# shanglianlm0525/CvPytorch

Measured on AMD Instinct MI355X. Metric: images/sec/node train step, YOLOv5-s@640 (value: batch resident in HBM when the timed region starts; with_h2d.value: the same step fed from pinned host memory inside the region) & DeepLabv3+R50@1024x512 (config3_deeplabv3plus_r50.value), higher is better.
Workload: dtype bf16; 1 GPU; coco_yolov5_s.yml YOLOv5-s 640x640 bf16 train step (fwd+loss+bwd+SGD-nesterov+EMA), per-GPU batch 64, synthetic COCO-shape tensors resident in HBM; global_batch=64, parallelism=dp1, launch=hipGraph replay of the whole step, world=1, transport=none (single process), grad_buckets=0, sync_bn=False, deterministic=True

## Files before the change

### cvpytorch_amd/csrc/conv1x1_stream.hip

```cpp
#include <stdlib.h>

#include "common.h"
#include "conv_plan.h"

namespace cvhip {

constexpr int kS1MaxLds = 72 * 1024;
constexpr int kS1MaxBlocks = 512;
constexpr int kS1MinTiles = 192;


template <int NV>
__device__ __forceinline__ void s1_act_vec(float (&v)[NV], int act, float ap) {
  switch (act) {
    case CVHIP_ACT_NONE: break;
    case CVHIP_ACT_RELU:
#pragma unroll
      for (int q = 0; q < NV; ++q) v[q] = act_fwd(v[q], CVHIP_ACT_RELU, ap);
      break;
    case CVHIP_ACT_SILU:
#pragma unroll
      for (int q = 0; q < NV; ++q) v[q] = act_fwd(v[q], CVHIP_ACT_SILU, ap);
      break;
    case CVHIP_ACT_LEAKY:
#pragma unroll
      for (int q = 0; q < NV; ++q) v[q] = act_fwd(v[q], CVHIP_ACT_LEAKY, ap);
      break;
    case CVHIP_ACT_SIGMOID:
#pragma unroll
      for (int q = 0; q < NV; ++q) v[q] = act_fwd(v[q], CVHIP_ACT_SIGMOID, ap);
      break;
    default:
#pragma unroll
      for (int q = 0; q < NV; ++q) v[q] = act_fwd(v[q], CVHIP_ACT_HSWISH, ap);
      break;
  }
}

template <int NF, int MF, int STATS, bool EPI = false, bool PRO = false>
__global__ __launch_bounds__(256, 2) void conv1x1_stream_kernel(const IgemmKernArgs p, int ntiles, int vec16) {
  constexpr int BN = NF * 16;
  constexpr int RT = 64 * MF;
  constexpr int KC = 256 / MF;
  constexpr int KS = KC / 32;
  extern __shared__ __attribute__((aligned(16))) unsigned char smem[];

  const int t = threadIdx.x;
  const int lane = t & 63;
  const int wave = __builtin_amdgcn_readfirstlane(t >> 6);
  const int r = lane & 15, g = lane >> 4;
  const int Cin = p.Cin;
  const int M = p.cls[0].M;
  const int cin_pad = (Cin + 31) & ~31;
  const int brow = cin_pad * 2 + 16;
  const int nkc = (cin_pad + KC - 1) / KC;
  const int n0 = blockIdx.y * BN;

  const int my_tiles = (ntiles - (int)blockIdx.x + (int)gridDim.x - 1) / (int)gridDim.x;
  const int total = my_tiles * nkc;

  h16x8 buf0[MF][KS], buf1[MF][KS];

  int ld_tile = blockIdx.x, ld_kc = 0;
  auto load = [&](h16x8 (&dst)[MF][KS]) {
    const int row0 = ld_tile * RT + wave * (MF * 16) + r;
    const int kbase = ld_kc * KC + g * 8;
#pragma unroll
    for (int b = 0; b < MF; ++b) {
      int m = row0 + b * 16;
      m = m < M ? m : M - 1;
      const h16_t* src = p.x + (int64_t)m * p.x_ld;
#pragma unroll
      for (int ks = 0; ks < KS; ++ks) {
        int kk = kbase + ks * 32;
        kk = kk < Cin ? kk : 0;
        dst[b][ks] = *reinterpret_cast<const h16x8*>(src + kk);
      }
    }
    if (++ld_kc == nkc) {
      ld_kc = 0;
      ld_tile += gridDim.x;
    }
  };

  load(buf0);

  {
    const int cpr = cin_pad >> 3;
    const int nchunks = BN * cpr;
    constexpr int U = 8;
    for (int q0 = t; q0 < nchunks; q0 += 256 * U) {
      uint4 v[U];
      int dst[U];
#pragma unroll
      for (int u = 0; u < U; ++u) {
        const int q = q0 + u * 256;
        const int L = q / cpr;
        const int kq = q - L * cpr;
        const int a = L >> 4, i = L & 15;
        const int ch = n0 + (a >> 1) * 32 + (i >> 2) * 8 + (a & 1) * 4 + (i & 3);
        dst[u] = q < nchunks ? L * brow + kq * 16 : -1;
        v[u] = make_uint4(0u, 0u, 0u, 0u);
        if (q < nchunks && ch < p.Nout && kq * 8 < Cin) v[u] = *reinterpret_cast<const uint4*>(p.w + (int64_t)ch * Cin + kq * 8);
      }
#pragma unroll
      for (int u = 0; u < U; ++u)
        if (dst[u] >= 0) *reinterpret_cast<uint4*>(smem + dst[u]) = v[u];
    }
  }
  float* const sbias = reinterpret_cast<float*>(smem + BN * brow);
  const float* const sepi = sbias + BN;
  if (p.bias && t < BN) sbias[t] = (n0 + t < p.bias_n) ? p.bias[n0 + t] : 0.f;
  static_assert(!EPI || STATS == 0, "the fused epilogue excludes BatchNorm sums");
  if (EPI && t < BN) {
    const int n = n0 + t < p.Nout ? n0 + t : p.Nout - 1;
    sbias[BN + t] = p.ep_scale ? p.ep_scale[n] : 1.f;
    sbias[2 * BN + t] = p.ep_scale ? p.ep_shift[n] : 0.f;
  }
  float* const spro = sbias + 5 * BN;
  if constexpr (PRO) {
    for (int c = t; c < cin_pad; c += 256) {
      const bool in = c >= p.pro_lo && c < p.pro_hi && c < Cin;
      spro[c] = in ? p.pro_scale[c] : 1.f;
      spro[cin_pad + c] = in ? p.pro_shift[c] : 0.f;
    }
  }
  __syncthreads();

  f32x4 acc[NF][MF];
#pragma unroll
  for (int a = 0; a < NF; ++a)
#pragma unroll
    for (int b = 0; b < MF; ++b) acc[a][b] = f32x4{0.f, 0.f, 0.f, 0.f};
  float s1[STATS ? NF : 1][4], s2[STATS ? NF : 1][4];
  if constexpr (STATS) {
#pragma unroll
    for (int a = 0; a < NF; ++a)
#pragma unroll
      for (int q = 0; q < 4; ++q) s1[a][q] = s2[a][q] = 0.f;
  }

  const unsigned char* const wlane = smem + r * brow + g * 16;
  int cp_tile = blockIdx.x, cp_kc = 0;
  auto compute = [&](const h16x8 (&src)[MF][KS]) {
    const unsigned char* wk = wlane + cp_kc * (KC * 2);
    const int ksn = min(KS, (cin_pad - cp_kc * KC) >> 5);
#pragma unroll
    for (int ks = 0; ks < KS; ++ks) {
      if (ks < ksn) {
#pragma unroll
        for (int a = 0; a < NF; ++a) {
          const h16x8 wb = *reinterpret_cast<const h16x8*>(wk + a * 16 * brow + ks * 64);
#pragma unroll
          for (int b = 0; b < MF; ++b) acc[a][b] = CVHIP_MFMA_16X16X32(wb, src[b][ks], acc[a][b], 0, 0, 0);
        }
      }
    }
    if (++cp_kc < nkc) return;
    const int row0 = cp_tile * RT + wave * (MF * 16) + r;
#pragma unroll
    for (int b = 0; b < MF; ++b) {
      const int m = row0 + b * 16;
      h16_t* yrow = p.y + (int64_t)m * p.y_ld;
#pragma unroll
      for (int j = 0; j < NF / 2; ++j) {
        const int ch0 = n0 + j * 32 + g * 8;
        f32x8 v;
#pragma unroll
        for (int q = 0; q < 4; ++q) {
          v.v[q] = acc[2 * j][b][q];
          v.v[4 + q] = acc[2 * j + 1][b][q];
        }
        if constexpr (STATS == 1) {
          const float keep = m < M ? 1.f : 0.f;
#pragma unroll
          for (int q = 0; q < 8; ++q) v.v[q] *= keep;
#pragma unroll
          for (int q = 0; q < 4; ++q) {
            s1[2 * j][q] += v.v[q];
            s2[2 * j][q] += v.v[q] * v.v[q];
            s1[2 * j + 1][q] += v.v[4 + q];
            s2[2 * j + 1][q] += v.v[4 + q] * v.v[4 + q];
          }
        }
        if (p.bias) {
          const f32x4 b0 = *reinterpret_cast<const f32x4*>(sbias + j * 32 + g * 8);
          const f32x4 b1 = *reinterpret_cast<const f32x4*>(sbias + j * 32 + g * 8 + 4);
#pragma unroll
          for (int q = 0; q < 4; ++q) {
            v.v[q] += b0[q];
            v.v[4 + q] += b1[q];
          }
        }
        if constexpr (EPI) {
          const int cl8 = j * 32 + g * 8;
#pragma unroll
          for (int q = 0; q < 8; ++q) v.v[q] = v.v[q] * sepi[cl8 + q] + sepi[BN + cl8 + q];
          if (p.res && p.res_pre && m < M) {
            const h16_t* rrow = p.res + (int64_t)m * p.res_ld + ch0;
#pragma unroll
            for (int q = 0; q < 8; ++q)
              if (ch0 + q < p.Nout) v.v[q] += (float)rrow[q];
          }
          s1_act_vec<8>(v.v, p.ep_act, p.ep_ap);
        }
        if (p.res && !(EPI && p.res_pre) && m < M) {
          const h16_t* rrow = p.res + (int64_t)m * p.res_ld + ch0;
          if (ch0 + 7 < p.Nout && (p.res_ld & 7) == 0 && ((((uintptr_t)p.res) & 15) == 0)) {
            const f32x8 rv = unpack8(*reinterpret_cast<const uint4*>(rrow));
#pragma unroll
            for (int q = 0; q < 8; ++q) v.v[q] += rv.v[q];
          } else {
#pragma unroll
            for (int q = 0; q < 8; ++q)
              if (ch0 + q < p.Nout) v.v[q] += (float)rrow[q];
          }
        }
        if (m < M) {
          h16_t* const dst = (p.y2 && ch0 >= p.y_split) ? p.y2 + (int64_t)m * p.y2_ld + (ch0 - p.y_split) : yrow + ch0;
          if (vec16 && ch0 + 7 < p.Nout) {
            *reinterpret_cast<uint4*>(dst) = pack8(v);
          } else {
#pragma unroll
            for (int q = 0; q < 8; ++q)
              if (ch0 + q < p.Nout) dst[q] = (h16_t)v.v[q];
          }
        }
      }
    }
#pragma unroll
    for (int a = 0; a < NF; ++a)
#pragma unroll
      for (int b = 0; b < MF; ++b) acc[a][b] = f32x4{0.f, 0.f, 0.f, 0.f};
    cp_kc = 0;
    cp_tile += gridDim.x;
  };

  auto xform = [&](h16x8 (&buf)[MF][KS]) {
    const int kbase = cp_kc * KC + g * 8;
    const int ksn = min(KS, (cin_pad - cp_kc * KC) >> 5);
#pragma unroll
    for (int ks = 0; ks < KS; ++ks) {
      int kk = kbase + ks * 32;
      kk = kk < Cin ? kk : 0;
      if (ks < ksn && kk >= p.pro_lo && kk < p.pro_hi) {
        const f32x4 c0 = *reinterpret_cast<const f32x4*>(spro + kk), c1 = *reinterpret_cast<const f32x4*>(spro + kk + 4);
        const f32x4 h0 = *reinterpret_cast<const f32x4*>(spro + cin_pad + kk), h1 = *reinterpret_cast<const f32x4*>(spro + cin_pad + kk + 4);
#pragma unroll
        for (int b = 0; b < MF; ++b) {
          f32x8 v = unpack8(__builtin_bit_cast(uint4, buf[b][ks]));
#pragma unroll
          for (int q = 0; q < 4; ++q) {
            v.v[q] = v.v[q] * c0[q] + h0[q];
            v.v[4 + q] = v.v[4 + q] * c1[q] + h1[q];
          }
          s1_act_vec<8>(v.v, p.pro_act, p.pro_ap);
          buf[b][ks] = __builtin_bit_cast(h16x8, pack8(v));
        }
      }
    }
  };

  for (int it = 0; it < total; it += 2) {
    load(buf1);
    if constexpr (PRO) xform(buf0);
    compute(buf0);
    load(buf0);
    if constexpr (PRO) xform(buf1);
    compute(buf1);
  }

  if constexpr (STATS) {
    if (p.stats) {
      __syncthreads();
      float* red = reinterpret_cast<float*>(smem);
#pragma unroll
      for (int a = 0; a < NF; ++a)
#pragma unroll
        for (int q = 0; q < 4; ++q) {
          const float u1 = row16_sum(s1[a][q]), u2 = row16_sum(s2[a][q]);
          if (r == 0) {
            const int lc = (a >> 1) * 32 + g * 8 + (a & 1) * 4 + q;
            red[(wave * BN + lc) * 2 + 0] = u1;
            red[(wave * BN + lc) * 2 + 1] = u2;
          }
        }
      __syncthreads();
      if (t < BN && n0 + t < p.Nout) {
        float u1 = 0.f, u2 = 0.f;
#pragma unroll
        for (int w = 0; w < 4; ++w) {
          u1 += red[(w * BN + t) * 2 + 0];
          u2 += red[(w * BN + t) * 2 + 1];
        }
        if (p.stats_acc) {
          acc_add2(reinterpret_cast<double*>(p.stats), blockIdx.x, p.stats_ld, n0 + t, u1, u2);
        } else {
          float* dst = p.stats + (int64_t)blockIdx.x * 2 * p.Nout;
          dst[n0 + t] = u1;
          dst[p.Nout + n0 + t] = u2;
        }
      }
    }
  }
}


static int s1x1_mode() {
  static int v = -1;
  if (v < 0) {
    const char* e = getenv("CVHIP_S1X1");
    v = e ? atoi(e) : 1;
  }
  return v;
}

static int s1x1_nf(int Nout, int Cin, bool stats) {
  if (Nout <= 32) return 2;
  if (Nout <= 64) return 4;
  if (Nout > 128 && Nout <= 256 && !stats && 256 * (((Cin + 31) & ~31) * 2 + 16) <= kS1MaxLds) return 16;
  return 8;
}

int stream1x1_blocks(int Nout, int Cin, int64_t M, bool stats) {
  const int mode = s1x1_mode();
  if (mode == 0 || (Cin & 7) || M <= 0 || M >= (1ll << 31)) return 0;
  const int bn = s1x1_nf(Nout, Cin, stats) * 16;
  const int cin_pad = (Cin + 31) & ~31;
  if (bn * (cin_pad * 2 + 16) > kS1MaxLds) return 0;
  const int ntiles = (int)((M + 127) / 128);
  if (mode == 1) {
    if (ntiles < kS1MinTiles) return 0;
    if (Nout > bn && (Nout > 4 * bn || stats || (double)M * Cin * 2.0 > 64e6)) return 0;
  }
  const int max_blocks = kS1MaxBlocks;
  const int rounds = cdiv(ntiles, max_blocks);
  return cdiv(ntiles, rounds);
}

static bool s1x1_structural(const IgemmParams& p) {
  if (p.ncls != 1) return false;
  const IgemmClass& c = p.cls[0];
  return c.TR == 1 && c.TS == 1 && p.in_sh == 1 && p.in_sw == 1 && p.out_sh == 1 && p.out_sw == 1 && c.dh0 == 0 && c.dw0 == 0 &&
         c.out_oh == 0 && c.out_ow == 0 && c.OHi == p.OH && c.OWi == p.OW && p.IH == p.OH && p.IW == p.OW && (p.x_ld & 7) == 0;
}

static int s1x1_lds(int bn, int cin_pad, bool pro) {
  int lds = bn * (cin_pad * 2 + 16) + 5 * bn * (int)sizeof(float) + (pro ? 2 * cin_pad * (int)sizeof(float) : 0);
  if (lds < 4 * bn * 2 * (int)sizeof(float)) lds = 4 * bn * 2 * (int)sizeof(float);
  return lds;
}
constexpr int kS1MaxLdsPro = kS1MaxLds + 4096;

template <int NF, int STATS, bool EPI = false, bool PRO = false>
static int launch_s1(const IgemmParams& p, int blocks, int ntiles, hipStream_t stream) {
  constexpr int MF = 2;
  const int bn = NF * 16;
  const int cin_pad = (p.Cin + 31) & ~31;
  const int lds = s1x1_lds(bn, cin_pad, PRO);
  if (lds > kS1MaxLdsPro) return CVHIP_ERR_UNSUPPORTED;
  auto kern = conv1x1_stream_kernel<NF, MF, STATS, EPI, PRO>;
  static bool attr_done[64] = {};
  int devid = 0;
  (void)hipGetDevice(&devid);
  bool& attr_set = attr_done[devid & 63];
  if (!attr_set) {
    hipError_t e = hipFuncSetAttribute(reinterpret_cast<const void*>(kern), hipFuncAttributeMaxDynamicSharedMemorySize, kS1MaxLds + 4096);
    if (e != hipSuccess) {
      set_last_error("hipFuncSetAttribute(conv1x1_stream_kernel)", e);
      return CVHIP_ERR_LAUNCH;
    }
    attr_set = true;
  }
  const int vec16 = ((p.y_ld & 7) == 0) && ((((uintptr_t)p.y) & 15) == 0);
  const IgemmKernArgs k = narrow_plan(p, 0, 1);
  hipLaunchKernelGGL(kern, dim3(blocks, cdiv(p.Nout, bn)), dim3(256), lds, stream, k, ntiles, vec16);
  return check_launch("conv1x1_stream_kernel");
}

bool stream1x1_prologue_ok(const IgemmParams& p, bool stats) {
  if (!s1x1_structural(p)) return false;
  if (stream1x1_blocks(p.Nout, p.Cin, p.cls[0].M, stats) <= 0) return false;
  const int nf = s1x1_nf(p.Nout, p.Cin, stats);
  if (nf == 16) return false;
  return s1x1_lds(nf * 16, (p.Cin + 31) & ~31, true) <= kS1MaxLdsPro;
}

int try_launch_stream1x1(const IgemmParams& p, hipStream_t stream) {
  if (!s1x1_structural(p)) return -1;
  const int64_t M = p.cls[0].M;
  const int blocks = stream1x1_blocks(p.Nout, p.Cin, M, p.stats != nullptr);
  if (blocks <= 0) return -1;
  const int ntiles = (int)((M + 127) / 128);
  const int nf = s1x1_nf(p.Nout, p.Cin, p.stats != nullptr);
  if (p.stats && (p.ep_scale || p.ep_act != CVHIP_ACT_NONE)) return CVHIP_ERR_INVALID;
  if (p.z_out) return CVHIP_ERR_UNSUPPORTED;
  if (p.y2 && ((p.y_split & 7) || p.y_split <= 0 || p.y_split >= p.Nout || (p.y2_ld & 7) || (((uintptr_t)p.y2) & 15) || (p.y_ld & 7) ||
               (((uintptr_t)p.y) & 15) || (p.Nout & 7)))
    return CVHIP_ERR_INVALID;
  if (p.pro_scale) {
    if (p.ep_scale || p.ep_act != CVHIP_ACT_NONE || p.res || !stream1x1_prologue_ok(p, p.stats != nullptr)) return CVHIP_ERR_UNSUPPORTED;
    if (p.pro_lo < 0 || p.pro_hi > p.Cin || p.pro_lo >= p.pro_hi || (p.pro_lo & 7) || (p.pro_hi & 7)) return CVHIP_ERR_INVALID;
    if (p.stats) {
      if (nf == 2) return launch_s1<2, 1, false, true>(p, blocks, ntiles, stream);
      if (nf == 4) return launch_s1<4, 1, false, true>(p, blocks, ntiles, stream);
      return launch_s1<8, 1, false, true>(p, blocks, ntiles, stream);
    }
    if (nf == 2) return launch_s1<2, 0, false, true>(p, blocks, ntiles, stream);
    if (nf == 4) return launch_s1<4, 0, false, true>(p, blocks, ntiles, stream);
    return launch_s1<8, 0, false, true>(p, blocks, ntiles, stream);
  }
  if (p.stats) {
    if (nf == 2) return launch_s1<2, 1>(p, blocks, ntiles, stream);
    if (nf == 4) return launch_s1<4, 1>(p, blocks, ntiles, stream);
    return launch_s1<8, 1>(p, blocks, ntiles, stream);
  }
  if (p.ep_scale || p.ep_act != CVHIP_ACT_NONE) {
    if (nf == 2) return launch_s1<2, 0, true>(p, blocks, ntiles, stream);
    if (nf == 4) return launch_s1<4, 0, true>(p, blocks, ntiles, stream);
    if (nf == 16) return launch_s1<16, 0, true>(p, blocks, ntiles, stream);
    return launch_s1<8, 0, true>(p, blocks, ntiles, stream);
  }
  if (nf == 2) return launch_s1<2, 0>(p, blocks, ntiles, stream);
  if (nf == 4) return launch_s1<4, 0>(p, blocks, ntiles, stream);
  if (nf == 16) return launch_s1<16, 0>(p, blocks, ntiles, stream);
  return launch_s1<8, 0>(p, blocks, ntiles, stream);
}

}
```

### cvpytorch_amd/ops.py

```python
import ctypes as C

import torch

from . import lib as L

ACT_DTYPE = torch.bfloat16
_weights_epoch = 0
_stats_epoch = [0]


def set_precision(p):
    global ACT_DTYPE
    L.set_precision(p)
    ACT_DTYPE = torch.float16 if p == "fp16" else torch.bfloat16
    bump_weights_epoch()
    _desc_cache.clear()


def precision():
    return L.PRECISION


def bump_weights_epoch():
    global _weights_epoch
    _weights_epoch += 1


_STEM_IMAGE = __import__("os").environ.get("CVHIP_STEM_IMAGE", "1") != "0"
_EPI_FUSE = __import__("os").environ.get("CVHIP_EPI_FUSE", "1") != "0"
_BN_ACC = __import__("os").environ.get("CVHIP_BN_ACC", "1") != "0"
_DW_STATS = __import__("os").environ.get("CVHIP_DW_STATS", "1") != "0"
_BN_ACC_MAX_C = 2048
_acc_epoch = 0


_DETERMINISTIC = __import__("os").environ.get("CVHIP_DETERMINISTIC", "0") == "1"


def set_deterministic(flag=True):
    global _DETERMINISTIC
    _DETERMINISTIC = bool(flag)


def is_deterministic():
    return _DETERMINISTIC


def _wgrad(kname, geom, desc, x, dy, dst, accumulate, st):
    if _DETERMINISTIC:
        nb = L.load().cvhip_conv2d_wgrad_det_workspace_bytes(C.byref(desc))
        if nb < 0:
            L.check(int(nb), "cvhip_conv2d_wgrad_det_workspace_bytes")
        ws = torch.empty((max(int(nb), 16),), dtype=torch.uint8, device=x.device)
        _timed_call(kname, geom, "cvhip_conv2d_wgrad_det", C.byref(desc), x.data_ptr(), dy.data_ptr(), dst.data_ptr(), int(accumulate),
                    ws.data_ptr(), int(nb), st)
    else:
        _timed_call(kname, geom, "cvhip_conv2d_wgrad", C.byref(desc), x.data_ptr(), dy.data_ptr(), dst.data_ptr(), int(accumulate), st)


def bump_acc_epoch():
    global _acc_epoch
    _acc_epoch += 1


def _layer_acc(cfg, K, dev):
    owner = cfg.acc_owner
    if owner is not None:
        ent = owner.__dict__.get(cfg.acc_attr)
        if ent is not None and len(ent) >= 4 and ent[3] == id(owner) and ent[1] != ent[2][0] and ent[0].shape[-1] == K and ent[0].device == dev:
            ent[1] = ent[2][0]
            return ent[0][0], ent[0][1]
    t = zero_fill(torch.empty((2, L.BN_ACC_SHARDS, 2, K), dtype=torch.float64, device=dev))
    return t[0], t[1]


def _stream():
    return torch.cuda.current_stream().cuda_stream


_LAZY = __import__("os").environ.get("CVHIP_LAZY", "1") != "0"
_LAZY_ACTS = (L.ACT_NONE, L.ACT_RELU, L.ACT_LEAKY, L.ACT_SILU)


_OWNED_BACKWARD = [False]


def set_lazy(flag=True):
    global _LAZY
    _LAZY = bool(flag)


class LazyAct:
    __slots__ = ("scale", "shift", "act", "ap", "z", "lo", "hi")

    def __init__(self, scale, shift, act, ap, lo=0, hi=None):
        self.scale, self.shift, self.act, self.ap = scale, shift, int(act), float(ap)
        self.lo = int(lo)
        self.hi = int(hi) if hi is not None else self.lo + int(scale.numel())
        self.z = None

    def full(self, Cc):
        return self.lo == 0 and self.hi == Cc

    def scale_ptr(self):
        return self.scale.data_ptr() - 4 * self.lo

    def shift_ptr(self):
        return self.shift.data_ptr() - 4 * self.lo


def act_id_of(conv_module):
    fus = conv_module._fusable(True, True) if hasattr(conv_module, "_fusable") else None
    return fus[1][0] if fus is not None else -1


def lazy_of(t):
    return getattr(t, "_hip_lazy", None) if t is not None else None


_LAZY_META = frozenset((
    "size", "stride", "dim", "ndimension", "numel", "nelement", "data_ptr", "storage_offset", "is_contiguous", "element_size", "__len__",
    "shape", "device", "dtype", "is_cuda", "requires_grad", "grad_fn", "is_leaf", "layout", "names", "ndim", "_version", "_base", "grad",
    "is_floating_point", "is_complex", "get_device", "is_sparse", "is_quantized", "is_meta", "untyped_storage", "_is_view", "output_nr",
    "register_hook", "retain_grad", "retains_grad", "__hash__", "__repr__", "__format__", "_backward_hooks", "is_pinned", "is_shared"))


class LazyRaw(torch.Tensor):

    @classmethod
    def __torch_function__(cls, func, types, args=(), kwargs=None):
        kwargs = kwargs or {}
        name = getattr(func, "__name__", "")
        if name == "__get__" or name == "__set__":
            name = getattr(getattr(func, "__self__", None), "__name__", name)
        if name in _LAZY_META:
            with torch._C.DisableTorchFunctionSubclass():
                return func(*args, **kwargs)
        from torch.utils._pytree import tree_map

        def fix(a):
            if isinstance(a, LazyRaw):
                with torch._C.DisableTorchFunctionSubclass():
                    return materialize(a) if lazy_of(a) is not None else a.as_subclass(torch.Tensor)
            return a

        args, kwargs = tree_map(fix, args), tree_map(fix, kwargs)
        with torch._C.DisableTorchFunctionSubclass():
            return func(*args, **kwargs)


def tag_lazy(t, lz):
    with torch._C.DisableTorchFunctionSubclass():
        z = t.as_subclass(LazyRaw)
    z._hip_lazy = lz
    return z


class Materialize(torch.autograd.Function):

    @staticmethod
    def forward(ctx, y, lz):
        yy, y_ld = as_nhwc(y, lazy_ok=True)
        N, K, P, Q = yy.shape
        z = empty_nhwc(N, K, P, Q, yy.device)
        _materialize_into(yy, y_ld, z, K, lz)
        return z

    @staticmethod
    def backward(ctx, dz):
        return dz, None


def _materialize_into(x, x_ld, z, z_ld, lz):
    N, Cc, H, W = x.shape
    M = N * H * W
    st = _stream()
    if not lz.full(Cc):
        L.call("cvhip_copy2d", x.data_ptr(), x_ld, z.data_ptr(), z_ld, M, Cc, st)
    kh = lz.hi - lz.lo
    _timed_ew("bn_act_fwd(ew_kernel<0>)", 4.0 * M * kh, "cvhip_bn_act_fwd", x.data_ptr() + 2 * lz.lo, x_ld, z.data_ptr() + 2 * lz.lo, z_ld, M, kh,
              lz.scale.data_ptr(), lz.shift.data_ptr(), lz.act, lz.ap, None, 0, st)


def materialize(x):
    lz = lazy_of(x)
    if lz is None:
        return x
    if lz.z is None:
        lz.z = Materialize.apply(x, lz)
    return lz.z


def _lazy_in(lz):
    return L.LazyIn(lz.scale_ptr(), lz.shift_ptr(), lz.act, lz.ap, lz.lo, lz.hi)


class KernelTimer:

    def __init__(self):
        self.enabled = False
        self.records = []
        self.detail = []

    def reset(self):
        self.records = []
        self.detail = []

    def summary(self):
        out = {}
        for name, fl, by, e0, e1 in self.records:
            d = out.setdefault(name, dict(launches=0, ms=0.0, flops=0.0, bytes=0.0))
            d["launches"] += 1
            d["ms"] += e0.elapsed_time(e1)
            d["flops"] += fl
            d["bytes"] += by
        return out


TIMER = KernelTimer()


def _igemm_name(nout, m=0, ktot=0, pointwise=False, ld=0, stats=False):
    if pointwise and ld % 8 == 0 and L.load().cvhip_conv1x1_stream_blocks(nout, ktot, m, int(stats)) > 0:
        wide = nout > 128 and not stats and 256 * (((ktot + 31) // 32 * 32) * 2 + 16) <= 72 * 1024 and nout <= 256
        return "conv1x1_stream_kernel<%d>" % (32 if nout <= 32 else 64 if nout <= 64 else 256 if wide else 128)
    if nout <= 32:
        return "igemm_kernel<256,32,64,32>"
    if nout <= 64:
        return "igemm_kernel<256,64,64,64>"
    big = ktot >= 512 and ((m + 255) // 256) * ((nout + 127) // 128) >= 384
    return "igemm_kernel<256,128,128,64>" if big else "igemm_kernel<128,128,64,64>"


def _pointwise(R, S, cfg):
    return R == 1 and S == 1 and tuple(cfg.stride) == (1, 1) and tuple(cfg.pad) == (0, 0)


def _wgrad_name(k, r=3, s=3, c=0, m=0, desc=None):
    if desc is not None and L.load().cvhip_conv_stem_blocks(C.byref(desc)) > 0 and desc.y_ld % 8 == 0:
        return "stem_wgrad_kernel"
    tn = 32 if k <= 32 else 64 if k <= 64 else 128
    if r == 1 and s == 1 and float(m) * k * c <= 7.5e9:
        if k >= 256 and c >= 256:
            return "wgrad_kernel<128,64,64,2>"
        tn = 32
    return {32: "wgrad_kernel<32,32,32>", 64: "wgrad_kernel<64,32,64>", 128: "wgrad_kernel<128,64,64>"}[tn]


def _timed_call(kname, geom, fname, *args, passes=1, nbytes=None):
    if not TIMER.enabled:
        L.call(fname, *args)
        return
    N, Cc, H, W, K, R, S, P, Q = geom
    flops = 2.0 * N * P * Q * K * R * S * Cc * passes
    if nbytes is None:
        nbytes = 2.0 * (N * H * W * Cc + N * P * Q * K + K * R * S * Cc)
    if kname.startswith("igemm_kernel") and (fname.startswith("cvhip_conv2d_fprop") or fname.startswith("cvhip_conv2d_dgrad")):
        try:
            dg = 1 if fname.startswith("cvhip_conv2d_dgrad") else 0
            bb = (C.c_int32 * L.BAND_PLAN_INTS)()
            buf = (C.c_int32 * (L.PATCH_CLASS_INTS * 4))()
            if L.load().cvhip_conv2d_band_plan(args[0], dg, bb) > 0:
                kname = "conv_band_kernel<%d ch/wave>" % (16 * bb[0])
            elif L.load().cvhip_conv2d_patch_plan(args[0], dg, buf, 4) > 0:
                kname = "conv_patch_kernel<128>"
        except Exception:
            pass
    elif kname.startswith("wgrad_kernel") and fname == "cvhip_conv2d_wgrad":
        try:
            wb = (C.c_int32 * L.WGRAD_BAND_PLAN_INTS)()
            if L.load().cvhip_conv2d_wgrad_band_plan(args[0], wb) > 0:
                kname = "wgrad_band_kernel<%d>" % wb[0]
        except Exception:
            pass
    e0, e1 = torch.cuda.Event(enable_timing=True), torch.cuda.Event(enable_timing=True)
    e0.record()
    L.call(fname, *args)
    e1.record()
    TIMER.records.append((kname, flops, nbytes, e0, e1))
    TIMER.detail.append((fname, geom))



def _timed_ew(kname, nbytes, fname, *args):
    if not TIMER.enabled:
        L.call(fname, *args)
        return
    e0, e1 = torch.cuda.Event(enable_timing=True), torch.cuda.Event(enable_timing=True)
    e0.record()
    L.call(fname, *args)
    e1.record()
    TIMER.records.append((kname, 0.0, float(nbytes), e0, e1))
    TIMER.detail.append((fname, None))


def _ptr(t, off=0):
    return None if t is None else t.data_ptr() + off


def empty_nhwc(N, Cc, H, W, device, ld=None):
    if ld is None or ld == Cc:
        return torch.empty((N, Cc, H, W), dtype=ACT_DTYPE, device=device, memory_format=torch.channels_last)
    buf = torch.empty((N, H, W, ld), dtype=ACT_DTYPE, device=device)
    return buf.permute(0, 3, 1, 2)[:, :Cc]


def nhwc_ld(t):
    if t.dim() != 4 or t.dtype != ACT_DTYPE:
        return None
    N, Cc, H, W = t.shape
    sN, sC, sH, sW = t.stride()
    if Cc > 1 and sC != 1:
        return None
    ld = sW if W > 1 else (sH if H > 1 else (sN if N > 1 else max(Cc, 1)))
    if W > 1 and sW != ld:
        return None
    if H > 1 and sH != W * ld:
        return None
    if N > 1 and sN != H * W * ld:
        return None
    if ld < Cc:
        return None
    return ld


def as_nhwc(t, lazy_ok=False):
    if not t.is_cuda:
        raise L.CvhipError("cvpytorch_amd ops need CUDA/HIP tensors (no CPU fallback); got %s" % t.device)
    if not lazy_ok and getattr(t, "_hip_lazy", None) is not None:
        raise L.CvhipError("a lazy activation reached an op that does not transform on load (ops.materialize it first)")
    if t.dtype != ACT_DTYPE:
        t = t.to(ACT_DTYPE)
    ld = nhwc_ld(t)
    if ld is None:
        t = t.contiguous(memory_format=torch.channels_last)
        ld = nhwc_ld(t)
    return t, ld


_desc_cache = {}


def conv_desc(N, Cc, H, W, K, R, S, stride, pad, dil, groups, x_ld, y_ld, k_valid=0, c_valid=0):
    key = (N, Cc, H, W, K, R, S, stride, pad, dil, groups, x_ld, y_ld, k_valid, c_valid)
    d = _desc_cache.get(key)
    if d is None:
        d = L.ConvDesc(N, Cc, H, W, K, R, S, stride[0], stride[1], pad[0], pad[1], dil[0], dil[1], groups, x_ld, y_ld,
                       k_valid, c_valid)
        _desc_cache[key] = d
    return d


def conv_out_hw(H, W, R, S, stride, pad, dil):
    P = (H + 2 * pad[0] - dil[0] * (R - 1) - 1) // stride[0] + 1
    Q = (W + 2 * pad[1] - dil[1] * (S - 1) - 1) // stride[1] + 1
    return P, Q


def _round8(x):
    return (x + 7) // 8 * 8


def zero_fill(t):
    L.call("cvhip_zero_fill", t.data_ptr(), t.numel() * t.element_size(), _stream())
    return t


def _krsc_master(weight):
    w = weight.detach()
    if w.dtype != torch.float32:
        w = w.float()
    wk = w.permute(0, 2, 3, 1)
    return wk if wk.is_contiguous() else wk.contiguous()


class ConvState:

    def __init__(self):
        self.key = None
        self.w_fprop = None
        self._wf_buf = None
        self.w_dgrad = None
        self.rec = None

    def prepare(self, weight, pdesc, need_dgrad, vkey):
        key = (vkey, _weights_epoch, pdesc.key(), L.PRECISION)
        if self.key == key and self.w_fprop is not None and (self.w_dgrad is not None or not need_dgrad):
            return
        dev = weight.device
        master = _krsc_master(weight)
        lib = L.load()
        shape = (pdesc.K, pdesc.R, pdesc.S, pdesc.C)
        nf = int(lib.cvhip_conv2d_weight_image_elems(C.byref(pdesc), 0))
        if nf < 0:
            L.check(nf, "cvhip_conv2d_weight_image_elems")
        if (self.w_fprop is None or tuple(self.w_fprop.shape) != shape or self.w_fprop.device != dev or self.w_fprop.dtype != ACT_DTYPE
                or self._wf_buf is None or self._wf_buf.numel() != nf):
            self._wf_buf = torch.empty((nf,), dtype=ACT_DTYPE, device=dev)
            self.w_fprop = self._wf_buf[:shape[0] * shape[1] * shape[2] * shape[3]].view(shape)
            self.w_dgrad = None
        wd = None
        if need_dgrad:
            n = lib.cvhip_conv2d_weight_image_elems(C.byref(pdesc), 1)
            if n < 0:
                L.check(int(n), "cvhip_conv2d_weight_image_elems")
            n = max(int(n), 8)
            wd = self.w_dgrad if (self.w_dgrad is not None and self.w_dgrad.numel() == n) else torch.empty((n,), dtype=ACT_DTYPE, device=dev)
        L.call("cvhip_conv2d_prep_weights", C.byref(pdesc), master.data_ptr(), self.w_fprop.data_ptr(), _ptr(wd), _stream())
        self._master_ref = master
        if wd is not None:
            self.w_dgrad = wd
        self.key = key
        self.rec = (master.data_ptr(), pdesc, vkey) if master.data_ptr() == weight.data_ptr() else None


class PrepPlan:

    def __init__(self, states):
        lib = L.load()
        self.states = [s for s in states if s.rec is not None and s.w_fprop is not None]
        n = len(self.states)
        self.n = n
        if n == 0:
            return
        entries = (L.PrepEntry * n)()
        self.ptrs = []
        for e, s in zip(entries, self.states):
            master, pdesc, _ = s.rec
            C.memmove(C.byref(e.desc), C.byref(pdesc), C.sizeof(L.ConvDesc))
            e.master, e.w_fprop = master, s.w_fprop.data_ptr()
            e.w_dgrad = s.w_dgrad.data_ptr() if s.w_dgrad is not None else None
            self.ptrs.append((master, e.w_fprop, e.w_dgrad))
        item = lib.cvhip_prep_plan_item_bytes()
        host = torch.zeros((n * item,), dtype=torch.uint8)
        blocks = C.c_int32(0)
        L.call("cvhip_prep_plan_build", C.cast(entries, C.c_void_p), n, host.data_ptr(), C.byref(blocks))
        self.blocks = int(blocks.value)
        self.table = host.to(self.states[0].w_fprop.device)

    def valid(self):
        return all(s.rec is not None and s.w_fprop is not None and (s.rec[0], s.w_fprop.data_ptr(), s.w_dgrad.data_ptr() if s.w_dgrad is not None else None) == p
                   for s, p in zip(self.states, self.ptrs))

    def run(self):
        if self.n == 0:
            return
        L.call("cvhip_prep_plan_run", self.table.data_ptr(), self.n, self.blocks, _stream())
        for s in self.states:
            s.key = (s.rec[2], _weights_epoch, s.rec[1].key(), L.PRECISION)


def conv_states_of(model):
    out = []
    for m in model.modules():
        for name in ("_hip_state", "_hip_pair_state"):
            s = m.__dict__.get(name)
            if isinstance(s, ConvState):
                out.append(s)
    return out


class ConvCfg:
    __slots__ = ("stride", "pad", "dil", "groups", "act", "act_param", "has_bn", "bn_training", "momentum", "eps",
                 "state", "track", "vkey", "gw", "gb", "gg", "gbeta", "arena", "idx_w", "idx_b", "idx_bn", "sync", "out", "out_split", "dx_link", "res_link", "res_pre",
                 "acc_owner", "acc_attr", "no_grad", "lazy_out", "lazy_half1", "lazy_half2", "lazy_made", "lazy_made2", "in_lazy", "res_lazy")

    def __init__(self, stride, pad, dil, groups=1, act=L.ACT_NONE, act_param=0.0, has_bn=False, bn_training=True,
                 momentum=0.1, eps=1e-5, state=None, track=True):
        self.stride, self.pad, self.dil, self.groups = tuple(stride), tuple(pad), tuple(dil), groups
        self.act, self.act_param = act, float(act_param)
        self.has_bn, self.bn_training = has_bn, bn_training
        self.momentum, self.eps = float(momentum), float(eps)
        self.state = state if state is not None else ConvState()
        self.track = track
        self.vkey = None
        self.gw = self.gb = self.gg = self.gbeta = None
        self.arena, self.idx_w, self.idx_b, self.idx_bn = None, None, None, ()
        self.sync = None
        self.out = None
        self.out_split = None
        self.dx_link = None
        self.res_link = None
        self.res_pre = False
        self.acc_owner = None
        self.acc_attr = "_hip_acc"
        self.no_grad = False
        self.lazy_out = False
        self.lazy_half1 = False
        self.lazy_half2 = False
        self.lazy_made = None
        self.lazy_made2 = None
        self.in_lazy = None
        self.res_lazy = None


def _sync_fwd_totals(partial, rows, K, M, sync):
    comm, world = sync
    tot = torch.empty((1 + L.REDUCE_SCRATCH_ROWS, 2, K), dtype=torch.float32, device=partial.device)
    L.call("cvhip_bn_bwd_finalize", partial.data_ptr(), rows, K, tot[0, 1].data_ptr(), tot[0, 0].data_ptr(), None, None, _stream())
    comm.allreduce_(tot[0])
    return tot, 1, M * world


def _sync_bwd_sums(dgamma, dbeta, sync):
    comm, world = sync
    g = torch.stack([dgamma, dbeta])
    comm.allreduce_(g)
    g = g / world
    return g[0], g[1]


def _colreduce_rows(M, Cc):
    return L.load().cvhip_colreduce_rows(M, Cc)


class GradLink:
    __slots__ = ("_g", "ok", "consumed", "__weakref__")

    def __init__(self):
        self._g = None
        self.ok = False
        self.consumed = False

    @property
    def g(self):
        return self._g

# ... 1952 lines not shown
```

Measured before the change: 4962 images/sec.

## Add 8-wave wide-tile variants of streaming 1x1 conv kernel with larger LDS

Generalizes the streaming 1x1 conv kernel to 8-wave blocks, optionally splitting output channels across two wave groups, and adds a planner. The planner picks a 256-channel full-width tile with 148KB LDS for mid-size Cin, and a 256-row tile for Cin up to 512 that previously fell back to the generic igemm. It also software-pipelines LDS weight reads against MFMAs using sched_group_barrier hints. The intent is to widen the weight tile per block, keep more 1x1 convs on the streaming path, and cut repeated activation reads across column blocks. The cost is one block per CU and lower occupancy.

```diff
diff --git a/cvpytorch_amd/csrc/conv1x1_stream.hip b/cvpytorch_amd/csrc/conv1x1_stream.hip
--- a/cvpytorch_amd/csrc/conv1x1_stream.hip
+++ b/cvpytorch_amd/csrc/conv1x1_stream.hip
@@ -8,6 +8,8 @@
 constexpr int kS1MaxLds = 72 * 1024;
 constexpr int kS1MaxBlocks = 512;
 constexpr int kS1MinTiles = 192;
+constexpr int kS1WideLds = 148 * 1024;
+constexpr int kS1WideBlocks = 256;
 
 
 template <int NV>
@@ -37,17 +39,25 @@
   }
 }
 
-template <int NF, int MF, int STATS, bool EPI = false, bool PRO = false>
-__global__ __launch_bounds__(256, 2) void conv1x1_stream_kernel(const IgemmKernArgs p, int ntiles, int vec16) {
+template <int NF, int MF, int STATS, bool EPI = false, bool PRO = false, int WAVES = 4, int CG = 1>
+__global__ __launch_bounds__(WAVES * 64, WAVES == 4 ? 2 : 1) void conv1x1_stream_kernel(const IgemmKernArgs p, int ntiles, int vec16) {
+  static_assert((WAVES == 4 || WAVES == 8) && (CG == 1 || CG == 2) && NF % (2 * CG) == 0 && !(PRO && WAVES != 4), "block shape");
   constexpr int BN = NF * 16;
-  constexpr int RT = 64 * MF;
+  constexpr int NFW = NF / CG;
+  constexpr int RW = WAVES / CG;
+  constexpr int NT = WAVES * 64;
+  constexpr int RT = 16 * MF * RW;
+  constexpr bool kTight = WAVES == 4 && (NFW == 16 || (NFW == 8 && PRO && STATS));
+  constexpr int WD = kTight ? 0 : (NFW < 4 ? NFW : 4);
   constexpr int KC = 256 / MF;
   constexpr int KS = KC / 32;
   extern __shared__ __attribute__((aligned(16))) unsigned char smem[];
 
   const int t = threadIdx.x;
   const int lane = t & 63;
-  const int wave = __builtin_amdgcn_readfirstlane(t >> 6);
+  const int wave_id = __builtin_amdgcn_readfirstlane(t >> 6);
+  const int wave = CG > 1 ? wave_id % RW : wave_id;
+  const int cg0 = CG > 1 ? (wave_id / RW) * (NFW * 16) : 0;
   const int r = lane & 15, g = lane >> 4;
   const int Cin = p.Cin;
   const int M = p.cls[0].M;
@@ -89,12 +99,12 @@
     const int cpr = cin_pad >> 3;
     const int nchunks = BN * cpr;
     constexpr int U = 8;
-    for (int q0 = t; q0 < nchunks; q0 += 256 * U) {
+    for (int q0 = t; q0 < nchunks; q0 += NT * U) {
       uint4 v[U];
       int dst[U];
 #pragma unroll
       for (int u = 0; u < U; ++u) {
-        const int q = q0 + u * 256;
+        const int q = q0 + u * NT;
         const int L = q / cpr;
         const int kq = q - L * cpr;
         const int a = L >> 4, i = L & 15;
@@ -119,7 +129,7 @@
   }
   float* const spro = sbias + 5 * BN;
   if constexpr (PRO) {
-    for (int c = t; c < cin_pad; c += 256) {
+    for (int c = t; c < cin_pad; c += NT) {
       const bool in = c >= p.pro_lo && c < p.pro_hi && c < Cin;
       spro[c] = in ? p.pro_scale[c] : 1.f;
       spro[cin_pad + c] = in ? p.pro_shift[c] : 0.f;
@@ -127,20 +137,20 @@
   }
   __syncthreads();
 
-  f32x4 acc[NF][MF];
-#pragma unroll
-  for (int a = 0; a < NF; ++a)
+  f32x4 acc[NFW][MF];
+#pragma unroll
+  for (int a = 0; a < NFW; ++a)
 #pragma unroll
     for (int b = 0; b < MF; ++b) acc[a][b] = f32x4{0.f, 0.f, 0.f, 0.f};
-  float s1[STATS ? NF : 1][4], s2[STATS ? NF : 1][4];
+  float s1[STATS ? NFW : 1][4], s2[STATS ? NFW : 1][4];
   if constexpr (STATS) {
 #pragma unroll
-    for (int a = 0; a < NF; ++a)
+    for (int a = 0; a < NFW; ++a)
 #pragma unroll
       for (int q = 0; q < 4; ++q) s1[a][q] = s2[a][q] = 0.f;
   }
 
-  const unsigned char* const wlane = smem + r * brow + g * 16;
+  const unsigned char* const wlane = smem + (cg0 + r) * brow + g * 16;
   int cp_tile = blockIdx.x, cp_kc = 0;
   auto compute = [&](const h16x8 (&src)[MF][KS]) {
     const unsigned char* wk = wlane + cp_kc * (KC * 2);
@@ -148,11 +158,30 @@
 #pragma unroll
     for (int ks = 0; ks < KS; ++ks) {
       if (ks < ksn) {
-#pragma unroll
-        for (int a = 0; a < NF; ++a) {
-          const h16x8 wb = *reinterpret_cast<const h16x8*>(wk + a * 16 * brow + ks * 64);
-#pragma unroll
-          for (int b = 0; b < MF; ++b) acc[a][b] = CVHIP_MFMA_16X16X32(wb, src[b][ks], acc[a][b], 0, 0, 0);
+        if constexpr (WD > 0) {
+          h16x8 wb[NFW];
+#pragma unroll
+          for (int a = 0; a < WD; ++a) wb[a] = *reinterpret_cast<const h16x8*>(wk + a * 16 * brow + ks * 64);
+#pragma unroll
+          for (int a = 0; a < NFW; ++a) {
+            if (a + WD < NFW) wb[a + WD] = *reinterpret_cast<const h16x8*>(wk + (a + WD) * 16 * brow + ks * 64);
+#pragma unroll
+            for (int b = 0; b < MF; ++b) acc[a][b] = CVHIP_MFMA_16X16X32(wb[a], src[b][ks], acc[a][b], 0, 0, 0);
+          }
+          __builtin_amdgcn_sched_group_barrier(0x100, WD, 0);
+#pragma unroll
+          for (int a = 0; a < NFW - WD; ++a) {
+            __builtin_amdgcn_sched_group_barrier(0x008, MF, 0);
+            __builtin_amdgcn_sched_group_barrier(0x100, 1, 0);
+          }
+          __builtin_amdgcn_sched_group_barrier(0x008, MF * WD, 0);
+        } else {
+#pragma unroll
+          for (int a = 0; a < NFW; ++a) {
+            const h16x8 wb = *reinterpret_cast<const h16x8*>(wk + a * 16 * brow + ks * 64);
+#pragma unroll
+            for (int b = 0; b < MF; ++b) acc[a][b] = CVHIP_MFMA_16X16X32(wb, src[b][ks], acc[a][b], 0, 0, 0);
+          }
         }
       }
     }
@@ -163,8 +192,9 @@
       const int m = row0 + b * 16;
       h16_t* yrow = p.y + (int64_t)m * p.y_ld;
 #pragma unroll
-      for (int j = 0; j < NF / 2; ++j) {
-        const int ch0 = n0 + j * 32 + g * 8;
+      for (int j = 0; j < NFW / 2; ++j) {
+        const int cl8 = cg0 + j * 32 + g * 8;
+        const int ch0 = n0 + cl8;
         f32x8 v;
 #pragma unroll
         for (int q = 0; q < 4; ++q) {
@@ -184,8 +214,8 @@
           }
         }
         if (p.bias) {
-          const f32x4 b0 = *reinterpret_cast<const f32x4*>(sbias + j * 32 + g * 8);
-          const f32x4 b1 = *reinterpret_cast<const f32x4*>(sbias + j * 32 + g * 8 + 4);
+          const f32x4 b0 = *reinterpret_cast<const f32x4*>(sbias + cl8);
+          const f32x4 b1 = *reinterpret_cast<const f32x4*>(sbias + cl8 + 4);
 #pragma unroll
           for (int q = 0; q < 4; ++q) {
             v.v[q] += b0[q];
@@ -193,7 +223,6 @@
           }
         }
         if constexpr (EPI) {
-          const int cl8 = j * 32 + g * 8;
 #pragma unroll
           for (int q = 0; q < 8; ++q) v.v[q] = v.v[q] * sepi[cl8 + q] + sepi[BN + cl8 + q];
           if (p.res && p.res_pre && m < M) {
@@ -229,7 +258,7 @@
       }
     }
 #pragma unroll
-    for (int a = 0; a < NF; ++a)
+    for (int a = 0; a < NFW; ++a)
 #pragma unroll
       for (int b = 0; b < MF; ++b) acc[a][b] = f32x4{0.f, 0.f, 0.f, 0.f};
     cp_kc = 0;
@@ -275,12 +304,12 @@
       __syncthreads();
       float* red = reinterpret_cast<float*>(smem);
 #pragma unroll
-      for (int a = 0; a < NF; ++a)
+      for (int a = 0; a < NFW; ++a)
 #pragma unroll
         for (int q = 0; q < 4; ++q) {
           const float u1 = row16_sum(s1[a][q]), u2 = row16_sum(s2[a][q]);
           if (r == 0) {
-            const int lc = (a >> 1) * 32 + g * 8 + (a & 1) * 4 + q;
+            const int lc = cg0 + (a >> 1) * 32 + g * 8 + (a & 1) * 4 + q;
             red[(wave * BN + lc) * 2 + 0] = u1;
             red[(wave * BN + lc) * 2 + 1] = u2;
           }
@@ -289,7 +318,7 @@
       if (t < BN && n0 + t < p.Nout) {
         float u1 = 0.f, u2 = 0.f;
 #pragma unroll
-        for (int w = 0; w < 4; ++w) {
+        for (int w = 0; w < RW; ++w) {
           u1 += red[(w * BN + t) * 2 + 0];
           u2 += red[(w * BN + t) * 2 + 1];
         }
@@ -322,21 +351,56 @@
   return 8;
 }
 
-int stream1x1_blocks(int Nout, int Cin, int64_t M, bool stats) {
-  const int mode = s1x1_mode();
-  if (mode == 0 || (Cin & 7) || M <= 0 || M >= (1ll << 31)) return 0;
-  const int bn = s1x1_nf(Nout, Cin, stats) * 16;
-  const int cin_pad = (Cin + 31) & ~31;
-  if (bn * (cin_pad * 2 + 16) > kS1MaxLds) return 0;
-  const int ntiles = (int)((M + 127) / 128);
-  if (mode == 1) {
-    if (ntiles < kS1MinTiles) return 0;
-    if (Nout > bn && (Nout > 4 * bn || stats || (double)M * Cin * 2.0 > 64e6)) return 0;
-  }
-  const int max_blocks = kS1MaxBlocks;
+struct S1Plan {
+  int nf = 0;
+  int waves = 4;
+  bool full = false;
+  int rt = 128;
+  int blocks = 0;
+};
+
+static int s1x1_grid(int64_t M, int rt, int max_blocks) {
+  const int ntiles = (int)((M + rt - 1) / rt);
   const int rounds = cdiv(ntiles, max_blocks);
   return cdiv(ntiles, rounds);
 }
+
+static S1Plan s1x1_plan(int Nout, int Cin, int64_t M, bool stats, bool narrow_only = false) {
+  S1Plan pl;
+  const int mode = s1x1_mode();
+  if (mode == 0 || (Cin & 7) || M <= 0 || M >= (1ll << 31)) return pl;
+  const int cin_pad = (Cin + 31) & ~31;
+  const int brow = cin_pad * 2 + 16;
+  const int ntiles = (int)((M + 127) / 128);
+  if (mode == 1 && ntiles < kS1MinTiles) return pl;
+  if (!narrow_only && Nout > 128 && Nout <= 256 && cin_pad > 128 && cin_pad <= 256 &&
+      (stats || mode != 1 || ntiles >= 2 * kS1WideBlocks)) {
+    pl.nf = 16, pl.waves = 8, pl.full = true, pl.rt = 128;
+    pl.blocks = s1x1_grid(M, pl.rt, kS1WideBlocks);
+    return pl;
+  }
+  const int bn = s1x1_nf(Nout, Cin, stats) * 16;
+  if (bn * brow <= kS1MaxLds) {
+    if (mode == 1) {
+      if (Nout > bn && (Nout > 4 * bn || stats || (double)M * Cin * 2.0 > 64e6)) return pl;
+    }
+    pl.nf = bn / 16;
+    pl.blocks = s1x1_grid(M, pl.rt, kS1MaxBlocks);
+    return pl;
+  }
+  if (!narrow_only && bn == 128 && cin_pad > 256 && cin_pad <= 512) {
+    const int ncol = cdiv(Nout, bn);
+    if (mode == 1) {
+      if (ncol < 2 || ncol > 4 || (double)M * Cin * 2.0 > 64e6) return pl;
+    }
+    pl.nf = 8, pl.waves = 8, pl.rt = 256;
+    pl.blocks = s1x1_grid(M, pl.rt, kS1WideBlocks / (ncol < kS1WideBlocks ? ncol : kS1WideBlocks));
+    return pl;
+  }
+  return pl;
+}
+
+int stream1x1_blocks(int Nout, int Cin, int64_t M, bool stats) { return s1x1_plan(Nout, Cin, M, stats).blocks; }
 
 static bool s1x1_structural(const IgemmParams& p) {
   if (p.ncls != 1) return false;
@@ -345,27 +409,29 @@
          c.out_oh == 0 && c.out_ow == 0 && c.OHi == p.OH && c.OWi == p.OW && p.IH == p.OH && p.IW == p.OW && (p.x_ld & 7) == 0;
 }
 
-static int s1x1_lds(int bn, int cin_pad, bool pro) {
+static int s1x1_lds(int bn, int cin_pad, bool pro, int rw = 4) {
   int lds = bn * (cin_pad * 2 + 16) + 5 * bn * (int)sizeof(float) + (pro ? 2 * cin_pad * (int)sizeof(float) : 0);
-  if (lds < 4 * bn * 2 * (int)sizeof(float)) lds = 4 * bn * 2 * (int)sizeof(float);
+  if (lds < rw * bn * 2 * (int)sizeof(float)) lds = rw * bn * 2 * (int)sizeof(float);
   return lds;
 }
 constexpr int kS1MaxLdsPro = kS1MaxLds + 4096;
 
-template <int NF, int STATS, bool EPI = false, bool PRO = false>
-static int launch_s1(const IgemmParams& p, int blocks, int ntiles, hipStream_t stream) {
-  constexpr int MF = 2;
+template <int NF, int STATS, bool EPI = false, bool PRO = false, int WAVES = 4, int CG = 1, int MF = 2>
+static int launch_s1(const IgemmParams& p, int blocks, hipStream_t stream) {
+  constexpr int RT = 16 * MF * (WAVES / CG);
+  constexpr int grant = WAVES == 4 ? kS1MaxLdsPro : kS1WideLds;
   const int bn = NF * 16;
   const int cin_pad = (p.Cin + 31) & ~31;
-  const int lds = s1x1_lds(bn, cin_pad, PRO);
-  if (lds > kS1MaxLdsPro) return CVHIP_ERR_UNSUPPORTED;
-  auto kern = conv1x1_stream_kernel<NF, MF, STATS, EPI, PRO>;
+  const int lds = s1x1_lds(bn, cin_pad, PRO, WAVES / CG);
+  if (lds > grant) return CVHIP_ERR_UNSUPPORTED;
+  const int ntiles = (int)((p.cls[0].M + RT - 1) / RT);
+  auto kern = conv1x1_stream_kernel<NF, MF, STATS, EPI, PRO, WAVES, CG>;
   static bool attr_done[64] = {};
   int devid = 0;
   (void)hipGetDevice(&devid);
   bool& attr_set = attr_done[devid & 63];
   if (!attr_set) {
-    hipError_t e = hipFuncSetAttribute(reinterpret_cast<const void*>(kern), hipFuncAttributeMaxDynamicSharedMemorySize, kS1MaxLds + 4096);
+    hipError_t e = hipFuncSetAttribute(reinterpret_cast<const void*>(kern), hipFuncAttributeMaxDynamicSharedMemorySize, grant);
     if (e != hipSuccess) {
       set_last_error("hipFuncSetAttribute(conv1x1_stream_kernel)", e);
       return CVHIP_ERR_LAUNCH;
@@ -374,25 +440,24 @@
   }
   const int vec16 = ((p.y_ld & 7) == 0) && ((((uintptr_t)p.y) & 15) == 0);
   const IgemmKernArgs k = narrow_plan(p, 0, 1);
-  hipLaunchKernelGGL(kern, dim3(blocks, cdiv(p.Nout, bn)), dim3(256), lds, stream, k, ntiles, vec16);
+  hipLaunchKernelGGL(kern, dim3(blocks, cdiv(p.Nout, bn)), dim3(WAVES * 64), lds, stream, k, ntiles, vec16);
   return check_launch("conv1x1_stream_kernel");
 }
 
 bool stream1x1_prologue_ok(const IgemmParams& p, bool stats) {
   if (!s1x1_structural(p)) return false;
-  if (stream1x1_blocks(p.Nout, p.Cin, p.cls[0].M, stats) <= 0) return false;
-  const int nf = s1x1_nf(p.Nout, p.Cin, stats);
-  if (nf == 16) return false;
-  return s1x1_lds(nf * 16, (p.Cin + 31) & ~31, true) <= kS1MaxLdsPro;
+  const S1Plan pl = s1x1_plan(p.Nout, p.Cin, p.cls[0].M, stats, true);
+  if (pl.blocks <= 0) return false;
+  if (pl.nf == 16) return false;
+  return s1x1_lds(pl.nf * 16, (p.Cin + 31) & ~31, true) <= kS1MaxLdsPro;
 }
 
 int try_launch_stream1x1(const IgemmParams& p, hipStream_t stream) {
   if (!s1x1_structural(p)) return -1;
   const int64_t M = p.cls[0].M;
-  const int blocks = stream1x1_blocks(p.Nout, p.Cin, M, p.stats != nullptr);
+  const S1Plan pl = s1x1_plan(p.Nout, p.Cin, M, p.stats != nullptr, p.pro_scale != nullptr);
+  const int blocks = pl.blocks, nf = pl.nf;
   if (blocks <= 0) return -1;
-  const int ntiles = (int)((M + 127) / 128);
-  const int nf = s1x1_nf(p.Nout, p.Cin, p.stats != nullptr);
   if (p.stats && (p.ep_scale || p.ep_act != CVHIP_ACT_NONE)) return CVHIP_ERR_INVALID;
   if (p.z_out) return CVHIP_ERR_UNSUPPORTED;
   if (p.y2 && ((p.y_split & 7) || p.y_split <= 0 || p.y_split >= p.Nout || (p.y2_ld & 7) || (((uintptr_t)p.y2) & 15) || (p.y_ld & 7) ||
@@ -402,29 +467,40 @@
     if (p.ep_scale || p.ep_act != CVHIP_ACT_NONE || p.res || !stream1x1_prologue_ok(p, p.stats != nullptr)) return CVHIP_ERR_UNSUPPORTED;
     if (p.pro_lo < 0 || p.pro_hi > p.Cin || p.pro_lo >= p.pro_hi || (p.pro_lo & 7) || (p.pro_hi & 7)) return CVHIP_ERR_INVALID;
     if (p.stats) {
-      if (nf == 2) return launch_s1<2, 1, false, true>(p, blocks, ntiles, stream);
-      if (nf == 4) return launch_s1<4, 1, false, true>(p, blocks, ntiles, stream);
-      return launch_s1<8, 1, false, true>(p, blocks, ntiles, stream);
-    }
-    if (nf == 2) return launch_s1<2, 0, false, true>(p, blocks, ntiles, stream);
-    if (nf == 4) return launch_s1<4, 0, false, true>(p, blocks, ntiles, stream);
-    return launch_s1<8, 0, false, true>(p, blocks, ntiles, stream);
+      if (nf == 2) return launch_s1<2, 1, false, true>(p, blocks, stream);
+      if (nf == 4) return launch_s1<4, 1, false, true>(p, blocks, stream);
+      return launch_s1<8, 1, false, true>(p, blocks, stream);
+    }
+    if (nf == 2) return launch_s1<2, 0, false, true>(p, blocks, stream);
+    if (nf == 4) return launch_s1<4, 0, false, true>(p, blocks, stream);
+    return launch_s1<8, 0, false, true>(p, blocks, stream);
+  }
+  const bool epi = p.ep_scale || p.ep_act != CVHIP_ACT_NONE;
+  if (pl.waves == 8) {
+    if (pl.full) {
+      if (p.stats) return launch_s1<16, 1, false, false, 8, 2>(p, blocks, stream);
+      if (epi) return launch_s1<16, 0, true, false, 8, 1, 1>(p, blocks, stream);
+      return launch_s1<16, 0, false, false, 8, 1, 1>(p, blocks, stream);
+    }
+    if (p.stats) return launch_s1<8, 1, false, false, 8, 1>(p, blocks, stream);
+    if (epi) return launch_s1<8, 0, true, false, 8, 1>(p, blocks, stream);
+    return launch_s1<8, 0, false, false, 8, 1>(p, blocks, stream);
   }
   if (p.stats) {
-    if (nf == 2) return launch_s1<2, 1>(p, blocks, ntiles, stream);
-    if (nf == 4) return launch_s1<4, 1>(p, blocks, ntiles, stream);
-    return launch_s1<8, 1>(p, blocks, ntiles, stream);
-  }
-  if (p.ep_scale || p.ep_act != CVHIP_ACT_NONE) {
-    if (nf == 2) return launch_s1<2, 0, true>(p, blocks, ntiles, stream);
-    if (nf == 4) return launch_s1<4, 0, true>(p, blocks, ntiles, stream);
-    if (nf == 16) return launch_s1<16, 0, true>(p, blocks, ntiles, stream);
-    return launch_s1<8, 0, true>(p, blocks, ntiles, stream);
-  }
-  if (nf == 2) return launch_s1<2, 0>(p, blocks, ntiles, stream);
-  if (nf == 4) return launch_s1<4, 0>(p, blocks, ntiles, stream);
-  if (nf == 16) return launch_s1<16, 0>(p, blocks, ntiles, stream);
-  return launch_s1<8, 0>(p, blocks, ntiles, stream);
-}
-
-}
+    if (nf == 2) return launch_s1<2, 1>(p, blocks, stream);
+    if (nf == 4) return launch_s1<4, 1>(p, blocks, stream);
+    return launch_s1<8, 1>(p, blocks, stream);
+  }
+  if (epi) {
+    if (nf == 2) return launch_s1<2, 0, true>(p, blocks, stream);
+    if (nf == 4) return launch_s1<4, 0, true>(p, blocks, stream);
+    if (nf == 16) return launch_s1<16, 0, true>(p, blocks, stream);
+    return launch_s1<8, 0, true>(p, blocks, stream);
+  }
+  if (nf == 2) return launch_s1<2, 0>(p, blocks, stream);
+  if (nf == 4) return launch_s1<4, 0>(p, blocks, stream);
+  if (nf == 16) return launch_s1<16, 0>(p, blocks, stream);
+  return launch_s1<8, 0>(p, blocks, stream);
+}
+
+}
diff --git a/cvpytorch_amd/ops.py b/cvpytorch_amd/ops.py
--- a/cvpytorch_amd/ops.py
+++ b/cvpytorch_amd/ops.py
@@ -222,7 +222,12 @@
 
 def _igemm_name(nout, m=0, ktot=0, pointwise=False, ld=0, stats=False):
     if pointwise and ld % 8 == 0 and L.load().cvhip_conv1x1_stream_blocks(nout, ktot, m, int(stats)) > 0:
-        wide = nout > 128 and not stats and 256 * (((ktot + 31) // 32 * 32) * 2 + 16) <= 72 * 1024 and nout <= 256
+        cin_pad = (ktot + 31) // 32 * 32
+        if 128 < nout <= 256 and 128 < cin_pad <= 256 and (stats or m >= 512 * 128 - 127):
+            return "conv1x1_stream_kernel<256>x8w"
+        if nout > 64 and 128 * (cin_pad * 2 + 16) > 72 * 1024:
+            return "conv1x1_stream_kernel<128>x8w"
+        wide = nout > 128 and not stats and 256 * (cin_pad * 2 + 16) <= 72 * 1024 and nout <= 256
         return "conv1x1_stream_kernel<%d>" % (32 if nout <= 32 else 64 if nout <= 64 else 256 if wide else 128)
     if nout <= 32:
         return "igemm_kernel<256,32,64,32>"
```

Result: no change. 4977 images/sec, median of 4 (+0.3%).
